# EcohydrologyTeam/ClearWater-riverine

Hardware: NVIDIA B200
Metric: cell_timesteps_per_sec (higher is better)
Workload: dtype f64

## Files before the change

clearwater_riverine_b200/csrc/cwr_api.cu:

```cuda
#include "../../include/cwr.h"

#include <cuda_runtime.h>

#include <algorithm>
#include <cmath>
#include <cstdio>
#include <cstdlib>
#include <cstring>
#include <map>
#include <string>
#include <vector>

#include "cwr_kernels.cuh"
#include "cwr_small.cuh"
#include "cwr_topology.h"

using namespace cwr;

static thread_local std::string g_create_error;

struct cwr_handle {
    int device = 0;
    cudaStream_t stream = nullptr;
    cwr_options opt{};
// ... 28 lines not shown
    int rank = 0, world = 1;
    bool attached = false;
    char* d_slab = nullptr; size_t slab_bytes = 0;
    uint8_t* d_send_mask = nullptr; int32_t* d_send_rows = nullptr;
    std::vector<void*> peer_maps;
    std::vector<int32_t> f1_ref, f2_ref;
    int last_iters = 0;
    bool small_path = false;
    bool tiny = false;
    int tiny_rpt = 1;
    int max_optin_smem = 0;
    bool pdl = false;
    int chip_ns = 0;
    bool in_run = false;
    SmallStats* d_stats = nullptr; SmallStats* h_stats = nullptr;
    int num_sms = 148, grid_rows = 0, grid_edges = 0, grid_b = 0, max_grid = 0, grid_spmm = 0, grid_at = 0, grid_xrp = 0;
    DeviceModel M{};
    int32_t *d_ell_col = nullptr, *d_ell_code = nullptr, *d_f1p = nullptr, *d_f2p = nullptr;
    int32_t *d_bcell = nullptr, *d_bptr = nullptr, *d_bedge = nullptr, *d_eperm = nullptr, *d_einv = nullptr;
    int32_t *d_new_of_old = nullptr, *d_old_of_new = nullptr, *d_f1 = nullptr, *d_f2 = nullptr;
    float *d_adv = nullptr, *d_velg = nullptr, *d_flowg = nullptr, *d_vol = nullptr;
    double* d_cdiff = nullptr;
    double* d_bc = nullptr;
    double* d_state = nullptr;
    double* d_dist = nullptr;
    void* d_stage = nullptr; size_t stage_bytes = 0;
    cudaStream_t up_stream = nullptr; cudaEvent_t compute_mark = nullptr;
    std::vector<cudaEvent_t> up_done; std::vector<uint8_t> up_pending;
    void* d_stage_up = nullptr; size_t stage_up_bytes = 0;
    cudaStream_t out_stream = nullptr; cudaEvent_t ev_extract[2] = {nullptr, nullptr}, ev_copied[2] = {nullptr, nullptr};
    double* d_out[2] = {nullptr, nullptr}; size_t out_bytes[2] = {0, 0}; int out_next = 0; bool out_pending[2] = {false, false};
    StepParams* d_sp = nullptr;
    StepParams* d_sp_ring = nullptr; size_t sp_ring_cap = 0; std::vector<StepParams> sp_host;
    const StepParams* sp_ready = nullptr;
    HostMirror* h_mirror = nullptr; HostMirror* d_mirror = nullptr;
    SolverCtl* h_ctl = nullptr;
    double* h_sc = nullptr; int* h_flags = nullptr;
    int n_state_slots = 0;
    std::vector<double> dt;
    std::vector<int> slot_time;
    std::vector<std::vector<double>> initial_row;
    std::vector<uint8_t> inputs_set;
    std::vector<std::map<int, std::vector<std::pair<int32_t, double>>>> real_overrides;
    int computed_upto = 0;
    int flux_step = -1;
    int lhs_step = -1;
    bool have_geometry = false;
    int64_t launches = 0, iterations = 0;
    bool kin_on = false;
    int kin_steps = 0, kin_temp_k = -1, kin_grid_max = 0;
    double kin_temp_c = 20.0;
    KinStep* d_kin_steps = nullptr; KinYield* d_kin_yields = nullptr; KinState* d_kin_state = nullptr; double* d_kin_partials = nullptr;
    int kin_srcs = 0, kin_src_o2 = 0;
    KinSrc* d_kin_srcs = nullptr;
    std::vector<double> kin_decay_h, kin_yields_h, kin_source_h, kin_exchange_h;
    std::vector<int> kin_step_of, kin_src_of;
    int kin_facs = 0;
    KinFac* d_kin_facs = nullptr; int* d_kin_fptr = nullptr;
    bool kin_depth = false;
    double kin_min_depth = 0.0;
    std::vector<double> kin_area_h;
// ... 151 lines not shown
    return v.empty() ? cudaSuccess : cudaMemcpyAsync(d, v.data(), v.size() * sizeof(T), cudaMemcpyHostToDevice, h->stream);
}

static int upload_kin_area(cwr_handle* h) {
    std::vector<double> a(h->n);
    for (int i = 0; i < h->n; ++i) a[i] = h->kin_area_h[h->topo.old_of_new[i]];
    CK(cudaMemcpyAsync(h->d_kin_area, a.data(), a.size() * sizeof(double), cudaMemcpyHostToDevice, h->stream));
    return CWR_OK;
}

static int upload_topology(cwr_handle* h) {
    const Topology& tp = h->topo;
    CK(put(h, h->d_ell_col, tp.ell_col)); CK(put(h, h->d_ell_code, tp.ell_code));
    CK(put(h, h->d_f1p, tp.f1p)); CK(put(h, h->d_f2p, tp.f2p));
    CK(put(h, h->d_bcell, tp.bcell)); CK(put(h, h->d_bptr, tp.bptr)); CK(put(h, h->d_bedge, tp.bedge));
    CK(put(h, h->d_eperm, tp.eperm));
    std::vector<int32_t> einv(tp.E);
    for (int ep = 0; ep < tp.E; ++ep) einv[tp.eperm[ep]] = ep;
    CK(put(h, h->d_einv, einv));
    CK(put(h, h->d_new_of_old, tp.new_of_old)); CK(put(h, h->d_old_of_new, tp.old_of_new));
    CK(put(h, h->d_color_ptr, tp.color_ptr));
    CK(put(h, h->d_send_mask, tp.send_mask)); CK(put(h, h->d_send_rows, tp.send_rows));
    if (h->strips) {
        CK(put(h, h->d_strip_cptr, tp.strip_cptr)); CK(put(h, h->d_strip_nptr, tp.strip_nptr));
        if (tp.strip_nbr.size() > h->strip_nbr_cap) {
            CK(cudaStreamSynchronize(h->stream));
            if (h->d_strip_nbr) CK(cudaFree(h->d_strip_nbr));
            h->d_strip_nbr = nullptr;
            h->strip_nbr_cap = tp.strip_nbr.size() + tp.strip_nbr.size() / 4 + 16;
            CK(cudaMalloc((void**)&h->d_strip_nbr, h->strip_nbr_cap * sizeof(int32_t)));
// ... 289 lines not shown
            CK(cudaFuncSetAttribute(k_solve_chip<12, false, true>, cudaFuncAttributeMaxDynamicSharedMemorySize, max_optin - kTinyStaticSmem));
            CK(cudaFuncSetAttribute(k_solve_chip<14, false, false>, cudaFuncAttributeMaxDynamicSharedMemorySize, max_optin - kTinyStaticSmem));
            CK(cudaFuncSetAttribute(k_solve_chip<14, false, true>, cudaFuncAttributeMaxDynamicSharedMemorySize, max_optin - kTinyStaticSmem));
            CK(cudaFuncSetAttribute(k_solve_chip<8, true, false>, cudaFuncAttributeMaxDynamicSharedMemorySize, max_optin - kTinyStaticSmem));
            CK(cudaFuncSetAttribute(k_solve_chip<8, true, true>, cudaFuncAttributeMaxDynamicSharedMemorySize, max_optin - kTinyStaticSmem));
            CK(cudaFuncSetAttribute(k_solve_chip<12, true, false>, cudaFuncAttributeMaxDynamicSharedMemorySize, max_optin - kTinyStaticSmem));
            CK(cudaFuncSetAttribute(k_solve_chip<12, true, true>, cudaFuncAttributeMaxDynamicSharedMemorySize, max_optin - kTinyStaticSmem));
            CK(cudaFuncSetAttribute(k_solve_chip<14, true, false>, cudaFuncAttributeMaxDynamicSharedMemorySize, max_optin - kTinyStaticSmem));
            CK(cudaFuncSetAttribute(k_solve_chip<14, true, true>, cudaFuncAttributeMaxDynamicSharedMemorySize, max_optin - kTinyStaticSmem));
            h->max_optin_smem = max_optin;
            choose_chip(h);
        }
    }
    h->grid_rows = grid_for(tp.part_ptr[h->rank + 1] - tp.part_ptr[h->rank], kThreads / kc, h->max_grid);
    h->grid_edges = grid_for(E / h->world + 1, kThreads / kc, h->max_grid);
    h->grid_b = grid_for((int64_t)(tp.bcell.size() / h->world + 1) * K, kThreads, h->max_grid);

    CK(dalloc(h, &h->d_ell_col, tp.ell_col.size())); CK(dalloc(h, &h->d_ell_code, tp.ell_code.size()));
    CK(dalloc(h, &h->d_f1p, tp.f1p.size())); CK(dalloc(h, &h->d_f2p, tp.f2p.size()));
    CK(dalloc(h, &h->d_bcell, tp.bcell.size())); CK(dalloc(h, &h->d_bptr, tp.bptr.size())); CK(dalloc(h, &h->d_bedge, tp.bedge.size()));
    CK(dalloc(h, &h->d_eperm, (size_t)E)); CK(dalloc(h, &h->d_einv, (size_t)E));
    CK(dalloc(h, &h->d_new_of_old, (size_t)n)); CK(dalloc(h, &h->d_old_of_new, (size_t)n));
    CK(dalloc(h, &h->d_color_ptr, tp.color_ptr.size()));
    CK(dalloc(h, &h->d_send_mask, (size_t)n)); CK(dalloc(h, &h->d_send_rows, (size_t)n));
    if (h->strips) {
        CK(dalloc(h, &h->d_strip_cptr, tp.strip_cptr.size())); CK(dalloc(h, &h->d_strip_nptr, tp.strip_nptr.size()));
        CK(dalloc(h, &h->d_strip_flag, (size_t)h->n_strips * kFlagStride));
        CK(cudaMemsetAsync(h->d_strip_flag, 0, (size_t)h->n_strips * kFlagStride * sizeof(unsigned long long), h->stream));
        CK(dalloc(h, &h->d_strip_peers, tp.strip_peers.size()));
        if ((size_t)h->world * h->n_strips * kFlagStride * sizeof(unsigned long long) > kDdCtlBytes - kDdFlagOffset)
            FAIL(CWR_EINVAL, "too many strips for the flag mirrors of a domain decomposition");
    }
    {
        int rc = upload_topology(h);
        if (rc) return rc;
// ... 11 lines not shown
    h->n_state_slots = h->opt.keep_history ? T : 2;
    const bool need_precond_vectors = h->m_steps > 1 || h->small_path;
    const size_t vec_bytes = (nK * sizeof(double) + 255) & ~(size_t)255;
    h->slab_bytes = kDdCtlBytes + (need_precond_vectors ? 3 : 0) * vec_bytes + (size_t)h->n_state_slots * nK * sizeof(double);
    if (cudaMalloc((void**)&h->d_slab, h->slab_bytes) != cudaSuccess) {
        cudaGetLastError();
        FAIL(CWR_ENOMEM, "not enough device memory for the concentration history; set keep_history = 0");
    }
    h->allocs.push_back(h->d_slab);
    CK(cudaMemsetAsync(h->d_slab, 0, h->slab_bytes, h->stream));
    h->d_state = (double*)(h->d_slab + kDdCtlBytes + (need_precond_vectors ? 3 : 0) * vec_bytes);

    DeviceModel& M = h->M;
    M.n = n; M.K = K; M.E = E; M.E_int = tp.E_int; M.E_g = tp.E_g; M.G = h->G; M.nb = (int)tp.bcell.size();
    M.W = tp.W; M.ell_col = h->d_ell_col; M.ell_code = h->d_ell_code; M.f1p = h->d_f1p; M.f2p = h->d_f2p;
    M.bcell = h->d_bcell; M.bptr = h->d_bptr; M.bedge = h->d_bedge;
    M.rank = h->rank; M.world = h->world;
    M.send_mask = h->d_send_mask;
    M.dd = (DdCtl*)h->d_slab; M.sym_base = h->d_slab;
    for (int q = 0; q < kMaxRanks; ++q) M.peer_base[q] = nullptr;
    M.peer_base[h->rank] = h->d_slab;
    set_owned_ranges(h);
    CK(dalloc(h, &M.val, (size_t)n * tp.W)); CK(dalloc(h, &M.diag, (size_t)n)); CK(dalloc(h, &M.gdiag, (size_t)n));
    CK(cudaMemsetAsync(M.gdiag, 0, (size_t)n * sizeof(double), h->stream));
    double* ic = nullptr;
    CK(dalloc(h, &ic, nK)); CK(cudaMemsetAsync(ic, 0, nK * sizeof(double), h->stream));
    M.ic = ic;
    CK(dalloc(h, &M.b, nK)); CK(dalloc(h, &M.r, nK));
    CK(cudaMemsetAsync(M.b, 0, nK * sizeof(double), h->stream)); CK(cudaMemsetAsync(M.r, 0, nK * sizeof(double), h->stream));
    {
        double** vs[] = {&M.rhat, &M.p, &M.v, &M.tt};
        for (double** v : vs) { CK(dalloc(h, v, nK)); CK(cudaMemsetAsync(*v, 0, nK * sizeof(double), h->stream)); }
    }
    if (need_precond_vectors) {
        double* us;
        CK(dalloc(h, &us, nK));
        CK(cudaMemsetAsync(us, 0, nK * sizeof(double), h->stream));
        M.ph = h->d_slab + kDdCtlBytes; M.sh = h->d_slab + kDdCtlBytes + vec_bytes; M.tmp = h->d_slab + kDdCtlBytes + 2 * vec_bytes;
        M.us = us;
// ... 263 lines not shown
}

static int state_available(cwr_handle* h, int t) {
    if (t < 0 || t >= h->T) FAIL(CWR_EINVAL, "time index out of range");
    if (t > h->computed_upto) FAIL(CWR_EINVAL, "state at this time index has not been computed yet");
    if (!h->opt.keep_history && t < h->computed_upto - 1) FAIL(CWR_EINVAL, "state no longer on the device (keep_history = 0)");
    return CWR_OK;
}

int cwr_set_state(cwr_handle* h, int k, int t, const double* c) {
    if (!h) return CWR_EINVAL;
    if (!c) FAIL(CWR_EINVAL, "NULL array");
    if (k < 0 || k >= h->K) FAIL(CWR_EINVAL, "constituent index out of range");
    int rc = state_available(h, t);
    if (rc) return rc;
    CK(cudaSetDevice(h->device));
    rc = ensure_stage(h, (size_t)h->n * 8);
    if (rc) return rc;
    CK(cudaMemcpyAsync(h->d_stage, c, (size_t)h->n * 8, cudaMemcpyHostToDevice, h->stream));
    k_scatter_column<<<grid_for(h->n, kThreads, h->max_grid), kThreads, 0, h->stream>>>(
        state_slot(h, t), (const double*)h->d_stage, h->d_old_of_new, h->n, h->K, k);
    h->launches += 1;
    CK(cudaGetLastError());
    CK(cudaStreamSynchronize(h->stream));
    return CWR_OK;
}

int cwr_set_state_all(cwr_handle* h, int t, const double* c, const uint8_t* mask) {
    if (!h) return CWR_EINVAL;
    if (!c) FAIL(CWR_EINVAL, "NULL array");
    int rc = state_available(h, t);
    if (rc) return rc;
    CK(cudaSetDevice(h->device));
    const size_t nK = (size_t)h->n * h->K;
    rc = ensure_stage(h, nK * 8 + 256);
    if (rc) return rc;
    uint8_t* dmask = nullptr;
    CK(cudaMemcpyAsync(h->d_stage, c, nK * 8, cudaMemcpyHostToDevice, h->stream));
    if (mask) {
        dmask = (uint8_t*)h->d_stage + nK * 8;
        CK(cudaMemcpyAsync(dmask, mask, h->K, cudaMemcpyHostToDevice, h->stream));
    }
    k_scatter_all<<<grid_for((int64_t)nK, kThreads, h->max_grid), kThreads, 0, h->stream>>>(
        state_slot(h, t), (const double*)h->d_stage, dmask, h->d_new_of_old, h->n, h->K);
    h->launches += 1;
    CK(cudaGetLastError());
    CK(cudaStreamSynchronize(h->stream));
// ... 111 lines not shown
        else if ((f & FL_BREAKDOWN) && !(f & FL_CONVERGED) && status == CWR_OK) status = CWR_EBREAKDOWN;
        else if (!(f & FL_CONVERGED) && status == CWR_OK) status = CWR_ENOTCONVERGED;
    }
    if (h->h_ctl->singular) status = CWR_ESINGULAR;
    if (h->h_ctl->barrier_timeout) { h->err = "a grid barrier timed out"; return CWR_ECUDA; }
    if (h->world > 1) {
        int dd_timeout = 0;
        CK(cudaMemcpyAsync(&dd_timeout, &h->M.dd->timeout, sizeof(int), cudaMemcpyDeviceToHost, h->stream));
        CK(cudaStreamSynchronize(h->stream));
        if (dd_timeout) { h->err = "a peer rank did not answer (halo barrier / dot-product exchange timed out)"; return CWR_ECUDA; }
    }
    if (info) { info->iterations = total_iter; info->restarts = restarts; info->status = status; info->max_relres = worst; }
    return status;
}

static int solve_dc(cwr_handle* h, cwr_step_info* info, bool* fell_back) {
    DeviceModel& M = h->M;
    *fell_back = false;
    mark(h, CWR_FAM_SPMM_INIT);
    KC_DISPATCH(h->KC, (k_spmm<KC, VEC, MODE_INIT_DC, double><<<h->grid_spmm, kThreads, 0, h->stream>>>(M, nullptr, nullptr)));
    h->launches += 1;
    mark(h, -1);
    int ahead = std::max(1, h->last_cycles);
    h->h_ctl->all_done = 0;
    int rc = CWR_OK;
    int launched = 0;
    while (!h->h_ctl->all_done) {
        const int burst = ahead > 0 ? ahead : h->opt.check_every;
        ahead = 0;
        for (int i = 0; i < burst; ++i) {
            const void* z = precondition(h, M.r, M.ph, M.tmp, true);
            mark(h, CWR_FAM_DC_UPDATE);
            PT_DISPATCH((k_spmm<KC, VEC, MODE_DC, PT><<<h->grid_spmm, kThreads, 0, h->stream>>>(M, (const PT*)z, nullptr)));
            h->launches += 1;
            ++launched;
// ... 77 lines not shown
    CK(cudaGetLastError());
    if (h->in_run) {
        if (info) { info->iterations = 0; info->restarts = 0; info->status = CWR_OK; info->max_relres = 0.0; }
        return CWR_OK;
    }
    int status = read_small_stats(h, info);
    if (status != CWR_ECUDA) h->iterations += (int64_t)(h->h_stats->sum_iterations / (unsigned long long)h->K);
    return status;
}

static int find_slot(cwr_handle* h, int t) {
    const int s = t % h->C;
    return h->slot_time[s] == t ? s : -1;
}

static int patch_real_cells(cwr_handle* h, int t, int before_solve) {
    DeviceModel& M = h->M;
    h->ov_idx.clear(); h->ov_val.clear();
    for (int k = 0; k < h->K; ++k) {
        auto it = h->real_overrides[k].find(t);
        if (it == h->real_overrides[k].end()) continue;
        for (auto& cv : it->second)
            if (cv.first >= M.row_lo && cv.first < M.row_hi) {
                h->ov_idx.push_back((long long)cv.first * h->K + k);
                h->ov_val.push_back(cv.second);
            }
    }
    const size_t cnt = h->ov_idx.size();
    if (cnt == 0) return CWR_OK;
    if (cnt > h->ov_cap) {
        CK(cudaStreamSynchronize(h->stream));
        if (h->d_ov_idx) CK(cudaFree(h->d_ov_idx));
        if (h->d_ov_val) CK(cudaFree(h->d_ov_val));
        h->d_ov_idx = nullptr; h->d_ov_val = nullptr;
        h->ov_cap = cnt + cnt / 2 + 64;
        CK(cudaMalloc((void**)&h->d_ov_idx, h->ov_cap * sizeof(long long)));
        CK(cudaMalloc((void**)&h->d_ov_val, h->ov_cap * sizeof(double)));
    }
    CK(cudaMemcpyAsync(h->d_ov_idx, h->ov_idx.data(), cnt * sizeof(long long), cudaMemcpyHostToDevice, h->stream));
    CK(cudaMemcpyAsync(h->d_ov_val, h->ov_val.data(), cnt * sizeof(double), cudaMemcpyHostToDevice, h->stream));
    CK(launch_chain(h, k_patch_rows, grid_for((int64_t)cnt, kThreads, 64), kThreads, 0, M, (const long long*)h->d_ov_idx, (const double*)h->d_ov_val, (int)cnt, before_solve));
    h->launches += 1;
    return CWR_OK;
}

static int build_rhs(cwr_handle* h, int t, int accumulate) {
    DeviceModel& M = h->M;
    mark(h, CWR_FAM_RHS);
    KC_DISPATCH(h->KC, (launch_chain(h, k_rhs<KC, VEC>, h->grid_rows, kThreads, 0, M)));
    h->launches += 1;
    int rc = patch_real_cells(h, t, 1);
    if (rc) return rc;
    if (h->kin_on) {
        const int R = react_tile_rows(h->K);
        const int grid = grid_for((M.row_hi - M.row_lo + R - 1) / R, 1, h->kin_grid_max);
        auto* fn = h->kin_depth ? k_react<true, true> : h->kin_facs ? k_react<true> : k_react<false>;
        const int* fptr = h->kin_depth && !h->kin_facs ? h->d_kin_fptr0 : h->d_kin_fptr;
        CK(launch_chain(h, fn, grid, kThreads, react_smem_bytes(h->K) + react_src_smem_bytes(h->kin_srcs, h->kin_temp_k), M,
                        (const KinStep*)h->d_kin_steps, h->kin_steps, (const KinYield*)h->d_kin_yields, h->kin_temp_k, h->kin_temp_c,
                        (const KinSrc*)h->d_kin_srcs, h->kin_srcs, h->kin_src_o2, (const KinFac*)h->d_kin_facs,
                        fptr, h->d_kin_partials, h->d_kin_state, accumulate, (const double*)h->d_kin_area,
                        (const int*)h->d_kin_dflag, h->kin_min_depth));
        h->launches += 1;
    }
    if (M.b_hi - M.b_lo > 0) {
        CK(launch_chain(h, k_boundary_rhs, h->grid_b, kThreads, 0, M));
        h->launches += 1;
    }
    return halo_push(h, h->cur_x);
}

static StepParams step_params(cwr_handle* h, int t, int s0, int s1) {
    const int n = h->n, E = h->E, K = h->K, Eg = std::max(1, h->topo.E_g), G = std::max(1, h->G);
    StepParams p;
    p.adv_t = h->d_adv + (size_t)s0 * E; p.cdiff_t = h->d_cdiff + (size_t)s0 * E;
    p.vol_t = h->d_vol + (size_t)s0 * n; p.vol_t1 = h->d_vol + (size_t)s1 * n;
    p.adv_t1 = h->d_adv + (size_t)s1 * E; p.cdiff_t1 = h->d_cdiff + (size_t)s1 * E;
    p.velg_t1 = h->d_velg + (size_t)s1 * Eg;
    p.flowg_t = h->d_flowg + (size_t)s0 * Eg;
    p.bc_t1 = h->d_bc + (size_t)(t + 1) * G * K;
    p.state_t = state_slot(h, t); p.state_t1 = state_slot(h, t + 1);
// ... 6 lines not shown
    if (t < 0 || t + 1 >= h->T) FAIL(CWR_EINVAL, "cwr_step: t must satisfy 0 <= t < n_time - 1 (dt[n_time-1] is NaN)");
    if (t > h->computed_upto) FAIL(CWR_EINVAL, "cwr_step: c[t] has not been computed yet");
    if (!h->opt.keep_history && t < h->computed_upto - 1) FAIL(CWR_EINVAL, "cwr_step: c[t] no longer on the device");
    for (int k = 0; k < h->K; ++k)
        if (!h->inputs_set[k]) FAIL(CWR_EINVAL, "cwr_set_inputs has not been called for every constituent");
    const int s0 = find_slot(h, t), s1 = find_slot(h, t + 1);
    if (s0 < 0 || s1 < 0) FAIL(CWR_EINVAL, "hydrodynamic slices t and t+1 are not resident; call cwr_set_hydro");
    CK(cudaSetDevice(h->device));
    { int rcj = join_prefetch(h, s0); if (rcj) return rcj; rcj = join_prefetch(h, s1); if (rcj) return rcj; }
    const int64_t launches0 = h->launches;
    const StepParams p = step_params(h, t, s0, s1);
    DeviceModel& M = h->M;
    if (h->sp_ready) M.sp = const_cast<StepParams*>(h->sp_ready);
    else CK(launch_chain(h, k_set_step, 1, 1, 0, p, h->d_sp, M.ctl, h->world > 1 ? M.dd : (DdCtl*)nullptr));
    h->cur_x = p.state_t1;
    mark(h, CWR_FAM_ASSEMBLE);
    if (h->world > 1 && !h->attached) FAIL(CWR_EINVAL, "domain-decomposed handle: call cwr_dd_attach before stepping");
    const int nb_own = M.b_hi - M.b_lo;
    if (nb_own > 0) CK(launch_chain(h, k_boundary_diag, grid_for(nb_own, kThreads, h->max_grid), kThreads, 0, M));
    CK(launch_chain(h, k_assemble, grid_for(M.row_hi - M.row_lo, kThreads, h->max_grid), kThreads, 0, M));
    h->launches += 2 + (nb_own > 0);
    h->lhs_step = t;
    { int rc = build_rhs(h, t, 1); if (rc) return rc; }
    cwr_step_info local{};
    int status;
    if (h->small_path) status = solve_small(h, &local);
    else if (h->dc) {
        bool fell_back = false;
        status = solve_dc(h, &local, &fell_back);
        if (fell_back) {
            ++h->fallbacks;
            const int cycles = h->h_ctl->iter, sweeps = h->h_ctl->sweeps_done;
            CK(cudaMemsetAsync(&M.ctl->all_done, 0, 2 * sizeof(int), h->stream));
            h->last_iters = 0;
            { int rc = build_rhs(h, t, 0); if (rc) return rc; }
            status = solve(h, &local);
            local.restarts += 1 + cycles;
            local.sweeps = sweeps;
        }
    } else status = solve(h, &local);
    if (status == CWR_ECUDA) return status;
    { int rc = patch_real_cells(h, t + 1, 0); if (rc) return rc; }
    { int rc = halo_push(h, p.state_t1); if (rc) return rc; }
    if (M.want_flux) {
        mark(h, CWR_FAM_MASS_FLUX);
        KC_DISPATCH(h->KC, (launch_chain(h, k_mass_flux<KC, VEC>, h->grid_edges, kThreads, 0, M)));
        h->launches += 1;
        h->flux_step = t;
    }
    flush_profile(h);
    CK(cudaGetLastError());
    h->computed_upto = std::max(h->computed_upto, t + 1);
    if (!h->opt.keep_history) h->computed_upto = t + 1;
    local.n_launches = (int)(h->launches - launches0);
    if (info) *info = local;
    if (status != CWR_OK) {
        char buf[160];
// ... 564 lines not shown
            const double v = pr.second < 0 ? diag[i] : val[pr.second] * diag[i];
            if (pr.first == last) data[pos - 1] += v;
            else { indices[pos] = pr.first; data[pos] = v; ++pos; last = pr.first; }
        }
    }
    indptr[n] = (int32_t)pos;
    return CWR_OK;
}

int cwr_get_rhs(cwr_handle* h, int k, double* b) {
    if (!h) return CWR_EINVAL;
    if (!b) FAIL(CWR_EINVAL, "NULL array");
    if (k < 0 || k >= h->K) FAIL(CWR_EINVAL, "constituent index out of range");
    if (h->lhs_step < 0) FAIL(CWR_EINVAL, "no step taken yet");
    CK(cudaSetDevice(h->device));
    const int n = h->n, K = h->K;
    std::vector<double> bs((size_t)n * K), diag(n);
    CK(cudaMemcpyAsync(bs.data(), h->M.b, bs.size() * 8, cudaMemcpyDeviceToHost, h->stream));
    CK(cudaMemcpyAsync(diag.data(), h->M.diag, (size_t)n * 8, cudaMemcpyDeviceToHost, h->stream));
    CK(cudaStreamSynchronize(h->stream));
    for (int r0 = 0; r0 < n; ++r0) {
        const int i = h->topo.new_of_old[r0];
        b[r0] = bs[(size_t)i * K + k] * diag[i];
    }
    return CWR_OK;
}

int cwr_get_permutation(cwr_handle* h, int32_t* new_of_old) {
    if (!h) return CWR_EINVAL;
    if (!new_of_old) FAIL(CWR_EINVAL, "NULL array");
// ... 161 lines not shown
```

clearwater_riverine_b200/csrc/cwr_kernels.cuh:

```cuda
#pragma once
#include <cuda_runtime.h>
#include <stdint.h>

#include "cwr_topology.h"

namespace cwr {

constexpr int kThreads = 256;
constexpr int kMaxK = 128;
constexpr int kMaxDots = 4;
#ifndef CWR_SPMM_MIN_BLOCKS
#define CWR_SPMM_MIN_BLOCKS 4
#endif
#ifndef CWR_AT_MIN_BLOCKS
#define CWR_AT_MIN_BLOCKS 3
#endif

struct StepParams {
    const float* adv_t;
    const double* cdiff_t;
    const float* vol_t;
    const float* vol_t1;
    const float* adv_t1;
    const double* cdiff_t1;
// ... 49 lines not shown
struct DeviceModel {
    int n, K, E, E_int, E_g, G, nb, W;
    int row_lo, row_hi, ie_lo, ie_hi, ge_lo, ge_hi, b_lo, b_hi;
    int rank, world;
    unsigned nbr_mask;
    const uint8_t* send_mask;
    const int32_t* send_rows; int n_send;
    int halo_per_sweep;
    char* peer_base[kMaxRanks];
    char* sym_base;
    DdCtl* dd;
    const int32_t* ell_col;
    const int32_t* ell_code;
    const int32_t* f1p; const int32_t* f2p;
    const int32_t* bcell; const int32_t* bptr; const int32_t* bedge;
    const int32_t* color_ptr; int n_colors;
    const int32_t* strip_cptr; const int32_t* strip_nptr; const int32_t* strip_nbr;
    const uint8_t* strip_peers;
    unsigned long long* strip_flag;
    int n_strips, strip0;
    int us_from_producer;
    int sweep_f32;
    int dc_smin, dc_smax;
    double dc_floor;
    double* val;
    float* valf;
    double* diag;
    double* gdiag;
    const double* ic;
    double *b, *r, *rhat, *p, *v, *tt, *xc;
    void *ph, *sh, *tmp, *us;
    double* partials;
    double* sc;
    int* colflags;
    int* coliters;
    SolverCtl* ctl;
    const StepParams* sp;
    double* flux;
    double* bsum;
    double* vsum;
    double tol2;
    double diffusion_coefficient;
    int max_iter;
// ... 114 lines not shown
        float ad = __fmul_rn(area, Df);
        adv[ep] = a;
        cdiff[ep] = (double)ad / dist[e];
        if (ep >= E_int) { velg[ep - E_int] = u; flowg[ep - E_int] = q; }
    }
}

__global__ void k_dist(double* __restrict__ dist, const double* __restrict__ fx, const double* __restrict__ fy,
                       const int32_t* __restrict__ f1, const int32_t* __restrict__ f2, int E) {
    for (int e = blockIdx.x * blockDim.x + threadIdx.x; e < E; e += gridDim.x * blockDim.x) {
        double dx = fx[f1[e]] - fx[f2[e]], dy = fy[f1[e]] - fy[f2[e]];
        dist[e] = sqrt(__dadd_rn(__dmul_rn(dx, dx), __dmul_rn(dy, dy)));
    }
}

__global__ void k_boundary_diag(DeviceModel M) {
    pdl_enter();
    const StepParams& sp = *M.sp;
    for (int b = M.b_lo + blockIdx.x * blockDim.x + threadIdx.x; b < M.b_hi; b += gridDim.x * blockDim.x) {
        double s = 0.0;
        for (int j = M.bptr[b]; j < M.bptr[b + 1]; ++j) {
            int e = M.bedge[j];
            s += sp.cdiff_t[e] + fmax((double)sp.adv_t[e], 0.0);
        }
        M.gdiag[M.bcell[b]] = s;
    }
}

__global__ void __launch_bounds__(kThreads) k_assemble(DeviceModel M) {
    pdl_enter();
    const StepParams& sp = *M.sp;
    const double dt = sp.dt;
    const int W = M.W;
    for (int i = M.row_lo + blockIdx.x * blockDim.x + threadIdx.x; i < M.row_hi; i += gridDim.x * blockDim.x) {
        const float vol = sp.vol_t1[i];
        double diag = (vol == 0.f ? 1.0 : 0.0) + (double)vol / dt + M.gdiag[i];
        const int32_t* code = M.ell_code + (size_t)i * W;
        double* val = M.val + (size_t)i * W;
        if (W == 4) {
            const int4 c4 = *reinterpret_cast<const int4*>(code);
            const int cs[4] = {c4.x, c4.y, c4.z, c4.w};
            double a[4], d[4], off[4];
#pragma unroll
            for (int u = 0; u < 4; ++u) {
                a[u] = cs[u] >= 0 ? (double)sp.adv_t[cs[u] >> 1] : 0.0;
                d[u] = cs[u] >= 0 ? sp.cdiff_t[cs[u] >> 1] : 0.0;
            }
#pragma unroll
            for (int u = 0; u < 4; ++u) {
                off[u] = 0.0;
                if (cs[u] >= 0) {
// ... 43 lines not shown
template <int VEC> struct Vd { double a[VEC]; };

template <int VEC>
__device__ __forceinline__ Vd<VEC> ldv(const double* p) {
    Vd<VEC> r;
    if (VEC == 2) { const double2 t = *reinterpret_cast<const double2*>(p); r.a[0] = t.x; r.a[VEC - 1] = t.y; }
    else r.a[0] = *p;
    return r;
}
template <int VEC>
__device__ __forceinline__ void stv(double* p, const Vd<VEC>& v) {
    if (VEC == 2) *reinterpret_cast<double2*>(p) = make_double2(v.a[0], v.a[VEC - 1]);
    else *p = v.a[0];
}

template <int KC, int VEC>
__global__ void __launch_bounds__(kThreads) k_rhs(DeviceModel M) {
    pdl_enter();
    const StepParams& sp = *M.sp;
    const int K = M.K, lane = threadIdx.x % KC, group = threadIdx.x / KC, GPB = kThreads / KC;
    const double dt = sp.dt;
    for (int c = lane * VEC; c < K; c += KC * VEC)
        for (int i = M.row_lo + blockIdx.x * GPB + group; i < M.row_hi; i += gridDim.x * GPB) {
            const size_t idx = (size_t)i * K + c;
            Vd<VEC> conc = ldv<VEC>(sp.state_t + idx);
            if (sp.apply_ic) {
                const Vd<VEC> ic = ldv<VEC>(M.ic + idx);
#pragma unroll
                for (int q = 0; q < VEC; ++q) if (ic.a[q] != 0.0) conc.a[q] = ic.a[q];
            }
            const double vol = (double)sp.vol_t[i], dg = M.diag[i];
            Vd<VEC> bb;
#pragma unroll
            for (int q = 0; q < VEC; ++q) bb.a[q] = (vol * conc.a[q] / dt) / dg;
            stv<VEC>(M.b + idx, bb);
            stv<VEC>(sp.state_t1 + idx, conc);
        }
}

__global__ void k_patch_rows(DeviceModel M, const long long* __restrict__ idx, const double* __restrict__ val, int count, int before_solve) {
    pdl_enter();
    const StepParams& sp = *M.sp;
    for (int q = blockIdx.x * blockDim.x + threadIdx.x; q < count; q += gridDim.x * blockDim.x) {
        const long long i = idx[q];
        const int row = (int)(i / M.K);
        sp.state_t1[i] = val[q];
        if (before_solve) M.b[i] = ((double)sp.vol_t[row] * val[q] / sp.dt) / M.diag[row];
    }
}

__global__ void __launch_bounds__(kThreads) k_boundary_rhs(DeviceModel M) {
    pdl_enter();
    const StepParams& sp = *M.sp;
    const int K = M.K;
    const double dt = sp.dt;
    const bool has_diffusion = M.diffusion_coefficient != 0.0;
    const size_t total = (size_t)(M.b_hi - M.b_lo) * K;
    for (size_t q = blockIdx.x * (size_t)blockDim.x + threadIdx.x; q < total; q += (size_t)gridDim.x * blockDim.x) {
        const int b = M.b_lo + (int)(q / K), c = (int)(q % K);
        const int i = M.bcell[b];
        double m_in = 0.0, ca_in = 0.0, cd_in = 0.0, m_out = 0.0, cd_out = 0.0;
        for (int j = M.bptr[b]; j < M.bptr[b + 1]; ++j) {
            const int e = M.bedge[j];
            const float u = sp.velg_t1[e - M.E_int];
            const double bc = sp.bc_t1[(size_t)(M.f2p[e] - M.n) * K + c];
            const double cd = has_diffusion ? fabs(sp.cdiff_t1[e]) : 0.0;
            if (u < 0.f) { m_in = bc; ca_in = fabs((double)sp.adv_t1[e]); cd_in = cd; }
            if (u > 0.f) { m_out = bc; cd_out = cd; }
        }
        const size_t idx = (size_t)i * K + c;
        const double conc = sp.state_t1[idx];
        const double load = (double)sp.vol_t[i] * conc / dt;
        const double rhs = load + (ca_in + cd_in) * m_in + cd_out * m_out;
        M.b[idx] = rhs / M.diag[i];
    }
}

template <int ND, int KC, int VEC>
__device__ __forceinline__ void block_dots(double (&acc)[ND * VEC], double* smem, double* partials, int K, int chunk) {
    constexpr int NA = ND * VEC;
#pragma unroll
    for (int off = KC; off < 32; off <<= 1)
#pragma unroll
        for (int d = 0; d < NA; ++d) acc[d] += __shfl_xor_sync(0xffffffffu, acc[d], off);
    const int wl = threadIdx.x & 31, warp = threadIdx.x >> 5;
    constexpr int NW = kThreads / 32;
    if (wl < KC)
#pragma unroll
        for (int d = 0; d < NA; ++d) smem[(warp * NA + d) * KC + wl] = acc[d];
    __syncthreads();
// ... 1142 lines not shown

template <int KC, int VEC, int MODE, typename ZT>
__global__ void __launch_bounds__(kThreads, MODE == 2 ? CWR_AT_MIN_BLOCKS : CWR_SPMM_MIN_BLOCKS) k_spmm(DeviceModel M, const ZT* __restrict__ zin,
                                                                        double* __restrict__ out) {
    constexpr bool IS_INIT = MODE == MODE_INIT || MODE == MODE_INIT_DC;
    constexpr int ND = IS_INIT ? 2 : MODE == MODE_AV ? 1 : MODE == MODE_AT ? 4 : 1;
    constexpr bool HAS_DOTS = IS_INIT || MODE == MODE_AV || MODE == MODE_AT || MODE == MODE_DC;
    __shared__ double smem[HAS_DOTS ? (kThreads / 32) * kMaxDots * 2 * 32 : 1];
    __shared__ double tot[HAS_DOTS ? kMaxDots * kMaxK : 1];
    if (MODE == MODE_AV || MODE == MODE_AT || MODE == MODE_DC) { if (M.ctl->all_done) return; }
    if (MODE == MODE_AT) { if (M.ctl->finish_half) return; }
    const int K = M.K, n = M.row_hi, W = M.W;
    const int lane = threadIdx.x % KC, group = threadIdx.x / KC, GPB = kThreads / KC;
    const int32_t* __restrict__ ecol = M.ell_col;
    const double* __restrict__ eval = M.val;
    if (IS_INIT) zin = reinterpret_cast<const ZT*>(M.sp->state_t1);
    double* __restrict__ xs = M.sp->state_t1;
    const int nchunk = (K + KC * VEC - 1) / (KC * VEC);
    for (int chunk = 0; chunk < nchunk; ++chunk) {
        const int c = (chunk * KC + lane) * VEC;
        const bool active = c < K;
        double acc[ND * VEC];
#pragma unroll
        for (int d = 0; d < ND * VEC; ++d) acc[d] = 0.0;
        if (active) {
            const int stride = gridDim.x * GPB;
            int i = M.row_lo + blockIdx.x * GPB + group;
            int4 c4n = make_int4(0, 0, 0, 0);
            double2 v01n = make_double2(0.0, 0.0), v23n = v01n;
            if (i < n) {
                c4n = *reinterpret_cast<const int4*>(ecol + (size_t)i * W);
                v01n = *reinterpret_cast<const double2*>(eval + (size_t)i * W);
                v23n = *reinterpret_cast<const double2*>(eval + (size_t)i * W + 2);
            }
            for (; i < n; i += stride) {
                const size_t idx = (size_t)i * K + c;
                const int4 c4 = make_int4(c4n.x & kColMask, c4n.y & kColMask, c4n.z & kColMask, c4n.w & kColMask);
                const double2 v01 = v01n, v23 = v23n;
                const Vd<VEC> x0 = ldz<ZT, VEC>(zin + (size_t)c4.x * K + c);
                const Vd<VEC> x1 = ldz<ZT, VEC>(zin + (size_t)c4.y * K + c);
                const Vd<VEC> x2 = ldz<ZT, VEC>(zin + (size_t)c4.z * K + c);
                const Vd<VEC> x3 = ldz<ZT, VEC>(zin + (size_t)c4.w * K + c);
                const Vd<VEC> own = ldz<ZT, VEC>(zin + idx);
                Vd<VEC> aux1 = own, aux2 = own;
                if (IS_INIT) aux1 = ldv<VEC>(M.b + idx);
                if (MODE == MODE_AV || MODE == MODE_AT) aux1 = ldv<VEC>(M.rhat + idx);
                if (MODE == MODE_DC) { aux1 = ldv<VEC>(M.r + idx); aux2 = ldv<VEC>(xs + idx); }
                if (MODE == MODE_AT) aux2 = ldv<VEC>(M.r + idx);
                const int inext = i + stride;
                if (inext < n) {
                    c4n = *reinterpret_cast<const int4*>(ecol + (size_t)inext * W);
                    v01n = *reinterpret_cast<const double2*>(eval + (size_t)inext * W);
                    v23n = *reinterpret_cast<const double2*>(eval + (size_t)inext * W + 2);
                }
                Vd<VEC> s;
#pragma unroll
                for (int q = 0; q < VEC; ++q)
                    s.a[q] = fma(v23.y, x3.a[q], fma(v23.x, x2.a[q], fma(v01.y, x1.a[q], v01.x * x0.a[q])));
                for (int w = 4; w < W; w += 4) {
                    int4 d4 = *reinterpret_cast<const int4*>(ecol + (size_t)i * W + w);
                    d4.x &= kColMask; d4.y &= kColMask; d4.z &= kColMask; d4.w &= kColMask;
                    const double2 w01 = *reinterpret_cast<const double2*>(eval + (size_t)i * W + w);
                    const double2 w23 = *reinterpret_cast<const double2*>(eval + (size_t)i * W + w + 2);
                    const Vd<VEC> y0 = ldz<ZT, VEC>(zin + (size_t)d4.x * K + c);
                    const Vd<VEC> y1 = ldz<ZT, VEC>(zin + (size_t)d4.y * K + c);
                    const Vd<VEC> y2 = ldz<ZT, VEC>(zin + (size_t)d4.z * K + c);
                    const Vd<VEC> y3 = ldz<ZT, VEC>(zin + (size_t)d4.w * K + c);
#pragma unroll
                    for (int q = 0; q < VEC; ++q)
                        s.a[q] = fma(w23.y, y3.a[q], fma(w23.x, y2.a[q], fma(w01.y, y1.a[q], fma(w01.x, y0.a[q], s.a[q]))));
                }
                Vd<VEC> y;
#pragma unroll
                for (int q = 0; q < VEC; ++q) y.a[q] = own.a[q] + s.a[q];
                if (IS_INIT) {
                    const Vd<VEC> bi = aux1;
                    Vd<VEC> r;
#pragma unroll
                    for (int q = 0; q < VEC; ++q) {
                        r.a[q] = bi.a[q] - y.a[q];
                        acc[0 * VEC + q] = fma(r.a[q], r.a[q], acc[0 * VEC + q]);
                        acc[1 * VEC + q] = fma(bi.a[q], bi.a[q], acc[1 * VEC + q]);
                    }
                    stv<VEC>(M.r + idx, r);
                    if (MODE == MODE_INIT) { stv<VEC>(M.rhat + idx, r); stv<VEC>(M.p + idx, r); }
                    if (MODE == MODE_INIT_DC && M.us_from_producer) {
                        if (M.sweep_f32) {
                            Pk<float, VEC> rs;
#pragma unroll
                            for (int q = 0; q < VEC; ++q) rs.a[q] = (float)r.a[q];
                            stk<float, VEC>(reinterpret_cast<float*>(M.us) + idx, rs);
                        } else stv<VEC>(reinterpret_cast<double*>(M.us) + idx, r);
                    }
                } else if (MODE == MODE_DC) {
                    Vd<VEC> r = aux1, xv = aux2;
#pragma unroll
                    for (int q = 0; q < VEC; ++q) {
                        r.a[q] -= y.a[q];
                        xv.a[q] += own.a[q];
                        acc[q] = fma(r.a[q], r.a[q], acc[q]);
                    }
                    stv<VEC>(M.r + idx, r); stv<VEC>(xs + idx, xv);
                    if (M.us_from_producer) {
                        Pk<ZT, VEC> rs;
#pragma unroll
                        for (int q = 0; q < VEC; ++q) rs.a[q] = (ZT)r.a[q];
                        stk<ZT, VEC>(reinterpret_cast<ZT*>(M.us) + idx, rs);
// ... 343 lines not shown
```

Measured before the change: 8.756 billion.

## Fuse RHS formation and boundary terms into assembly and DC initial SpMM

Removes the separate boundary-diagonal and boundary-RHS kernels. Ghost diagonal contributions are now computed inside k_assemble through a new cell-to-boundary-row map, and the RHS is formed on the fly in the MODE_INIT_DC SpMM from c[t] instead of being written to b and read back. On the direct path the state copy into t+1 is done by the SpMM itself, so several launches and one full pass over b and the state are dropped. In exchange cwr_get_rhs must recompute b lazily and fails if c[t] has been evicted, and edge-value prefetching is disabled in the init-DC mode.

```diff
diff --git a/clearwater_riverine_b200/csrc/cwr_api.cu b/clearwater_riverine_b200/csrc/cwr_api.cu
--- a/clearwater_riverine_b200/csrc/cwr_api.cu
+++ b/clearwater_riverine_b200/csrc/cwr_api.cu
@@ -66,10 +66,10 @@
     int chip_ns = 0;
     bool in_run = false;
     SmallStats* d_stats = nullptr; SmallStats* h_stats = nullptr;
-    int num_sms = 148, grid_rows = 0, grid_edges = 0, grid_b = 0, max_grid = 0, grid_spmm = 0, grid_at = 0, grid_xrp = 0;
+    int num_sms = 148, grid_rows = 0, grid_edges = 0, max_grid = 0, grid_spmm = 0, grid_at = 0, grid_xrp = 0;
     DeviceModel M{};
     int32_t *d_ell_col = nullptr, *d_ell_code = nullptr, *d_f1p = nullptr, *d_f2p = nullptr;
-    int32_t *d_bcell = nullptr, *d_bptr = nullptr, *d_bedge = nullptr, *d_eperm = nullptr, *d_einv = nullptr;
+    int32_t *d_bcell = nullptr, *d_bptr = nullptr, *d_bedge = nullptr, *d_brow = nullptr, *d_eperm = nullptr, *d_einv = nullptr;
     int32_t *d_new_of_old = nullptr, *d_old_of_new = nullptr, *d_f1 = nullptr, *d_f2 = nullptr;
     float *d_adv = nullptr, *d_velg = nullptr, *d_flowg = nullptr, *d_vol = nullptr;
     double* d_cdiff = nullptr;
@@ -97,6 +97,7 @@
     int computed_upto = 0;
     int flux_step = -1;
     int lhs_step = -1;
+    bool rhs_direct = false, rhs_lost = false;
     bool have_geometry = false;
     int64_t launches = 0, iterations = 0;
     bool kin_on = false;
@@ -278,6 +279,9 @@
     CK(put(h, h->d_ell_col, tp.ell_col)); CK(put(h, h->d_ell_code, tp.ell_code));
     CK(put(h, h->d_f1p, tp.f1p)); CK(put(h, h->d_f2p, tp.f2p));
     CK(put(h, h->d_bcell, tp.bcell)); CK(put(h, h->d_bptr, tp.bptr)); CK(put(h, h->d_bedge, tp.bedge));
+    std::vector<int32_t> brow(tp.n, -1);
+    for (size_t b = 0; b < tp.bcell.size(); ++b) brow[tp.bcell[b]] = (int32_t)b;
+    CK(put(h, h->d_brow, brow));
     CK(put(h, h->d_eperm, tp.eperm));
     std::vector<int32_t> einv(tp.E);
     for (int ep = 0; ep < tp.E; ++ep) einv[tp.eperm[ep]] = ep;
@@ -597,11 +601,11 @@
     }
     h->grid_rows = grid_for(tp.part_ptr[h->rank + 1] - tp.part_ptr[h->rank], kThreads / kc, h->max_grid);
     h->grid_edges = grid_for(E / h->world + 1, kThreads / kc, h->max_grid);
-    h->grid_b = grid_for((int64_t)(tp.bcell.size() / h->world + 1) * K, kThreads, h->max_grid);
 
     CK(dalloc(h, &h->d_ell_col, tp.ell_col.size())); CK(dalloc(h, &h->d_ell_code, tp.ell_code.size()));
     CK(dalloc(h, &h->d_f1p, tp.f1p.size())); CK(dalloc(h, &h->d_f2p, tp.f2p.size()));
     CK(dalloc(h, &h->d_bcell, tp.bcell.size())); CK(dalloc(h, &h->d_bptr, tp.bptr.size())); CK(dalloc(h, &h->d_bedge, tp.bedge.size()));
+    CK(dalloc(h, &h->d_brow, (size_t)tp.n));
     CK(dalloc(h, &h->d_eperm, (size_t)E)); CK(dalloc(h, &h->d_einv, (size_t)E));
     CK(dalloc(h, &h->d_new_of_old, (size_t)n)); CK(dalloc(h, &h->d_old_of_new, (size_t)n));
     CK(dalloc(h, &h->d_color_ptr, tp.color_ptr.size()));
@@ -643,15 +647,14 @@
     DeviceModel& M = h->M;
     M.n = n; M.K = K; M.E = E; M.E_int = tp.E_int; M.E_g = tp.E_g; M.G = h->G; M.nb = (int)tp.bcell.size();
     M.W = tp.W; M.ell_col = h->d_ell_col; M.ell_code = h->d_ell_code; M.f1p = h->d_f1p; M.f2p = h->d_f2p;
-    M.bcell = h->d_bcell; M.bptr = h->d_bptr; M.bedge = h->d_bedge;
+    M.bcell = h->d_bcell; M.bptr = h->d_bptr; M.bedge = h->d_bedge; M.brow = h->d_brow;
     M.rank = h->rank; M.world = h->world;
     M.send_mask = h->d_send_mask;
     M.dd = (DdCtl*)h->d_slab; M.sym_base = h->d_slab;
     for (int q = 0; q < kMaxRanks; ++q) M.peer_base[q] = nullptr;
     M.peer_base[h->rank] = h->d_slab;
     set_owned_ranges(h);
-    CK(dalloc(h, &M.val, (size_t)n * tp.W)); CK(dalloc(h, &M.diag, (size_t)n)); CK(dalloc(h, &M.gdiag, (size_t)n));
-    CK(cudaMemsetAsync(M.gdiag, 0, (size_t)n * sizeof(double), h->stream));
+    CK(dalloc(h, &M.val, (size_t)n * tp.W)); CK(dalloc(h, &M.diag, (size_t)n));
     double* ic = nullptr;
     CK(dalloc(h, &ic, nK)); CK(cudaMemsetAsync(ic, 0, nK * sizeof(double), h->stream));
     M.ic = ic;
@@ -945,6 +948,7 @@
     if (k < 0 || k >= h->K) FAIL(CWR_EINVAL, "constituent index out of range");
     int rc = state_available(h, t);
     if (rc) return rc;
+    if (t == h->lhs_step) h->rhs_lost = true;
     CK(cudaSetDevice(h->device));
     rc = ensure_stage(h, (size_t)h->n * 8);
     if (rc) return rc;
@@ -962,6 +966,7 @@
     if (!c) FAIL(CWR_EINVAL, "NULL array");
     int rc = state_available(h, t);
     if (rc) return rc;
+    if (t == h->lhs_step) h->rhs_lost = true;
     CK(cudaSetDevice(h->device));
     const size_t nK = (size_t)h->n * h->K;
     rc = ensure_stage(h, nK * 8 + 256);
@@ -1103,11 +1108,12 @@
     return status;
 }
 
-static int solve_dc(cwr_handle* h, cwr_step_info* info, bool* fell_back) {
+static int solve_dc(cwr_handle* h, cwr_step_info* info, bool* fell_back, const double* c_tilde) {
     DeviceModel& M = h->M;
     *fell_back = false;
     mark(h, CWR_FAM_SPMM_INIT);
-    KC_DISPATCH(h->KC, (k_spmm<KC, VEC, MODE_INIT_DC, double><<<h->grid_spmm, kThreads, 0, h->stream>>>(M, nullptr, nullptr)));
+    double* b_out = h->rhs_direct ? nullptr : M.b;
+    KC_DISPATCH(h->KC, (k_spmm<KC, VEC, MODE_INIT_DC, double><<<h->grid_spmm, kThreads, 0, h->stream>>>(M, c_tilde, b_out)));
     h->launches += 1;
     mark(h, -1);
     int ahead = std::max(1, h->last_cycles);
@@ -1215,7 +1221,7 @@
     return h->slot_time[s] == t ? s : -1;
 }
 
-static int patch_real_cells(cwr_handle* h, int t, int before_solve) {
+static int patch_real_cells(cwr_handle* h, int t) {
     DeviceModel& M = h->M;
     h->ov_idx.clear(); h->ov_val.clear();
     for (int k = 0; k < h->K; ++k) {
@@ -1240,17 +1246,27 @@
     }
     CK(cudaMemcpyAsync(h->d_ov_idx, h->ov_idx.data(), cnt * sizeof(long long), cudaMemcpyHostToDevice, h->stream));
     CK(cudaMemcpyAsync(h->d_ov_val, h->ov_val.data(), cnt * sizeof(double), cudaMemcpyHostToDevice, h->stream));
-    CK(launch_chain(h, k_patch_rows, grid_for((int64_t)cnt, kThreads, 64), kThreads, 0, M, (const long long*)h->d_ov_idx, (const double*)h->d_ov_val, (int)cnt, before_solve));
+    CK(launch_chain(h, k_patch_rows, grid_for((int64_t)cnt, kThreads, 64), kThreads, 0, M, (const long long*)h->d_ov_idx, (const double*)h->d_ov_val, (int)cnt));
     h->launches += 1;
     return CWR_OK;
 }
 
-static int build_rhs(cwr_handle* h, int t, int accumulate) {
+static bool has_real_overrides(const cwr_handle* h, int t) {
+    for (int k = 0; k < h->K; ++k)
+        if (h->real_overrides[k].count(t)) return true;
+    return false;
+}
+
+static int front_end(cwr_handle* h, int t, bool direct, bool form_b, int accumulate) {
     DeviceModel& M = h->M;
+    mark(h, CWR_FAM_ASSEMBLE);
+    CK(launch_chain(h, k_assemble, grid_for(M.row_hi - M.row_lo, kThreads, h->max_grid), kThreads, 0, M, direct ? 0 : 1));
+    h->launches += 1;
+    h->lhs_step = t;
+    h->rhs_direct = direct; h->rhs_lost = false;
+    if (direct) return CWR_OK;
     mark(h, CWR_FAM_RHS);
-    KC_DISPATCH(h->KC, (launch_chain(h, k_rhs<KC, VEC>, h->grid_rows, kThreads, 0, M)));
-    h->launches += 1;
-    int rc = patch_real_cells(h, t, 1);
+    int rc = patch_real_cells(h, t);
     if (rc) return rc;
     if (h->kin_on) {
         const int R = react_tile_rows(h->K);
@@ -1264,8 +1280,8 @@
                         (const int*)h->d_kin_dflag, h->kin_min_depth));
         h->launches += 1;
     }
-    if (M.b_hi - M.b_lo > 0) {
-        CK(launch_chain(h, k_boundary_rhs, h->grid_b, kThreads, 0, M));
+    if (form_b) {
+        KC_DISPATCH(h->KC, (launch_chain(h, k_rhs<KC, VEC>, h->grid_rows, kThreads, 0, M, (const double*)h->cur_x)));
         h->launches += 1;
     }
     return halo_push(h, h->cur_x);
@@ -1302,33 +1318,28 @@
     if (h->sp_ready) M.sp = const_cast<StepParams*>(h->sp_ready);
     else CK(launch_chain(h, k_set_step, 1, 1, 0, p, h->d_sp, M.ctl, h->world > 1 ? M.dd : (DdCtl*)nullptr));
     h->cur_x = p.state_t1;
-    mark(h, CWR_FAM_ASSEMBLE);
     if (h->world > 1 && !h->attached) FAIL(CWR_EINVAL, "domain-decomposed handle: call cwr_dd_attach before stepping");
-    const int nb_own = M.b_hi - M.b_lo;
-    if (nb_own > 0) CK(launch_chain(h, k_boundary_diag, grid_for(nb_own, kThreads, h->max_grid), kThreads, 0, M));
-    CK(launch_chain(h, k_assemble, grid_for(M.row_hi - M.row_lo, kThreads, h->max_grid), kThreads, 0, M));
-    h->launches += 2 + (nb_own > 0);
-    h->lhs_step = t;
-    { int rc = build_rhs(h, t, 1); if (rc) return rc; }
+    const bool direct = h->dc && h->world == 1 && t >= 1 && !h->kin_on && !has_real_overrides(h, t);
+    { int rc = front_end(h, t, direct, !h->dc, 1); if (rc) return rc; }
     cwr_step_info local{};
     int status;
     if (h->small_path) status = solve_small(h, &local);
     else if (h->dc) {
         bool fell_back = false;
-        status = solve_dc(h, &local, &fell_back);
+        status = solve_dc(h, &local, &fell_back, direct ? p.state_t : p.state_t1);
         if (fell_back) {
             ++h->fallbacks;
             const int cycles = h->h_ctl->iter, sweeps = h->h_ctl->sweeps_done;
             CK(cudaMemsetAsync(&M.ctl->all_done, 0, 2 * sizeof(int), h->stream));
             h->last_iters = 0;
-            { int rc = build_rhs(h, t, 0); if (rc) return rc; }
+            { int rc = front_end(h, t, false, true, 0); if (rc) return rc; }
             status = solve(h, &local);
             local.restarts += 1 + cycles;
             local.sweeps = sweeps;
         }
     } else status = solve(h, &local);
     if (status == CWR_ECUDA) return status;
-    { int rc = patch_real_cells(h, t + 1, 0); if (rc) return rc; }
+    { int rc = patch_real_cells(h, t + 1); if (rc) return rc; }
     { int rc = halo_push(h, p.state_t1); if (rc) return rc; }
     if (M.want_flux) {
         mark(h, CWR_FAM_MASS_FLUX);
@@ -1923,6 +1934,14 @@
     if (k < 0 || k >= h->K) FAIL(CWR_EINVAL, "constituent index out of range");
     if (h->lhs_step < 0) FAIL(CWR_EINVAL, "no step taken yet");
     CK(cudaSetDevice(h->device));
+    if (h->rhs_direct) {
+        const int t = h->lhs_step;
+        if (h->rhs_lost || state_available(h, t) != CWR_OK || find_slot(h, t) < 0 || find_slot(h, t + 1) < 0)
+            FAIL(CWR_EINVAL, "cwr_get_rhs: c[t] or the hydrodynamic slices t, t+1 of the last step are no longer on the device");
+        KC_DISPATCH(h->KC, (launch_chain(h, k_rhs<KC, VEC>, h->grid_rows, kThreads, 0, h->M, (const double*)state_slot(h, t))));
+        h->launches += 1;
+        CK(cudaGetLastError());
+    }
     const int n = h->n, K = h->K;
     std::vector<double> bs((size_t)n * K), diag(n);
     CK(cudaMemcpyAsync(bs.data(), h->M.b, bs.size() * 8, cudaMemcpyDeviceToHost, h->stream));
diff --git a/clearwater_riverine_b200/csrc/cwr_kernels.cuh b/clearwater_riverine_b200/csrc/cwr_kernels.cuh
--- a/clearwater_riverine_b200/csrc/cwr_kernels.cuh
+++ b/clearwater_riverine_b200/csrc/cwr_kernels.cuh
@@ -87,6 +87,7 @@
     const int32_t* ell_code;
     const int32_t* f1p; const int32_t* f2p;
     const int32_t* bcell; const int32_t* bptr; const int32_t* bedge;
+    const int32_t* brow;
     const int32_t* color_ptr; int n_colors;
     const int32_t* strip_cptr; const int32_t* strip_nptr; const int32_t* strip_nbr;
     const uint8_t* strip_peers;
@@ -99,7 +100,6 @@
     double* val;
     float* valf;
     double* diag;
-    double* gdiag;
     const double* ic;
     double *b, *r, *rhat, *p, *v, *tt, *xc;
     void *ph, *sh, *tmp, *us;
@@ -244,27 +244,38 @@
     }
 }
 
-__global__ void k_boundary_diag(DeviceModel M) {
-    pdl_enter();
-    const StepParams& sp = *M.sp;
-    for (int b = M.b_lo + blockIdx.x * blockDim.x + threadIdx.x; b < M.b_hi; b += gridDim.x * blockDim.x) {
-        double s = 0.0;
-        for (int j = M.bptr[b]; j < M.bptr[b + 1]; ++j) {
-            int e = M.bedge[j];
-            s += sp.cdiff_t[e] + fmax((double)sp.adv_t[e], 0.0);
-        }
-        M.gdiag[M.bcell[b]] = s;
-    }
-}
-
-__global__ void __launch_bounds__(kThreads) k_assemble(DeviceModel M) {
+__global__ void __launch_bounds__(kThreads) k_assemble(DeviceModel M, int with_x0) {
     pdl_enter();
     const StepParams& sp = *M.sp;
     const double dt = sp.dt;
     const int W = M.W;
+    if (with_x0) {
+        const size_t lo = (size_t)M.row_lo * M.K, hi = (size_t)M.row_hi * M.K, stride = (size_t)gridDim.x * blockDim.x;
+        const double* __restrict__ src = sp.state_t;
+        double* __restrict__ dst = sp.state_t1;
+        for (size_t q = lo + blockIdx.x * (size_t)blockDim.x + threadIdx.x; q < hi; q += 2 * stride) {
+            const size_t q1 = q + stride;
+            double v0 = src[q], v1 = q1 < hi ? src[q1] : 0.0;
+            if (sp.apply_ic) {
+                const double i0 = M.ic[q], i1 = q1 < hi ? M.ic[q1] : 0.0;
+                if (i0 != 0.0) v0 = i0;
+                if (i1 != 0.0) v1 = i1;
+            }
+            dst[q] = v0;
+            if (q1 < hi) dst[q1] = v1;
+        }
+    }
     for (int i = M.row_lo + blockIdx.x * blockDim.x + threadIdx.x; i < M.row_hi; i += gridDim.x * blockDim.x) {
         const float vol = sp.vol_t1[i];
-        double diag = (vol == 0.f ? 1.0 : 0.0) + (double)vol / dt + M.gdiag[i];
+        const double own = (vol == 0.f ? 1.0 : 0.0) + (double)vol / dt;
+        const int bi = M.brow[i];
+        double ghost = 0.0;
+        if (bi >= 0)
+            for (int j = M.bptr[bi]; j < M.bptr[bi + 1]; ++j) {
+                const int e = M.bedge[j];
+                ghost += sp.cdiff_t[e] + fmax((double)sp.adv_t[e], 0.0);
+            }
+        double diag = own + ghost;
         const int32_t* code = M.ell_code + (size_t)i * W;
         double* val = M.val + (size_t)i * W;
         if (W == 4) {
@@ -338,8 +349,44 @@
     else *p = v.a[0];
 }
 
+template <int VEC>
+__device__ __forceinline__ Vd<VEC> rhs_row(const DeviceModel& M, const StepParams& sp, int bi, int c, const Vd<VEC>& conc,
+                                           float vol, double dg, double dt) {
+    Vd<VEC> b;
+#pragma unroll
+    for (int q = 0; q < VEC; ++q) b.a[q] = __dmul_rn((double)vol, conc.a[q]) / dt;
+    if (bi >= 0) {
+        int e_in = -1, e_out = -1;
+        for (int j = M.bptr[bi]; j < M.bptr[bi + 1]; ++j) {
+            const int e = M.bedge[j];
+            const float u = sp.velg_t1[e - M.E_int];
+            if (u < 0.f) e_in = e;
+            if (u > 0.f) e_out = e;
+        }
+        const bool has_diffusion = M.diffusion_coefficient != 0.0;
+        double cin = 0.0, cd_out = 0.0;
+        const double* bc_in = nullptr; const double* bc_out = nullptr;
+        if (e_in >= 0) {
+            cin = __dadd_rn(fabs((double)sp.adv_t1[e_in]), has_diffusion ? fabs(sp.cdiff_t1[e_in]) : 0.0);
+            bc_in = sp.bc_t1 + (size_t)(M.f2p[e_in] - M.n) * M.K + c;
+        }
+        if (e_out >= 0) {
+            cd_out = has_diffusion ? fabs(sp.cdiff_t1[e_out]) : 0.0;
+            bc_out = sp.bc_t1 + (size_t)(M.f2p[e_out] - M.n) * M.K + c;
+        }
+#pragma unroll
+        for (int q = 0; q < VEC; ++q) {
+            const double m_in = bc_in ? bc_in[q] : 0.0, m_out = bc_out ? bc_out[q] : 0.0;
+            b.a[q] = __dadd_rn(__dadd_rn(b.a[q], __dmul_rn(cin, m_in)), __dmul_rn(cd_out, m_out));
+        }
+    }
+#pragma unroll
+    for (int q = 0; q < VEC; ++q) b.a[q] = b.a[q] / dg;
+    return b;
+}
+
 template <int KC, int VEC>
-__global__ void __launch_bounds__(kThreads) k_rhs(DeviceModel M) {
+__global__ void __launch_bounds__(kThreads) k_rhs(DeviceModel M, const double* __restrict__ src) {
     pdl_enter();
     const StepParams& sp = *M.sp;
     const int K = M.K, lane = threadIdx.x % KC, group = threadIdx.x / KC, GPB = kThreads / KC;
@@ -347,57 +394,15 @@
     for (int c = lane * VEC; c < K; c += KC * VEC)
         for (int i = M.row_lo + blockIdx.x * GPB + group; i < M.row_hi; i += gridDim.x * GPB) {
             const size_t idx = (size_t)i * K + c;
-            Vd<VEC> conc = ldv<VEC>(sp.state_t + idx);
-            if (sp.apply_ic) {
-                const Vd<VEC> ic = ldv<VEC>(M.ic + idx);
-#pragma unroll
-                for (int q = 0; q < VEC; ++q) if (ic.a[q] != 0.0) conc.a[q] = ic.a[q];
-            }
-            const double vol = (double)sp.vol_t[i], dg = M.diag[i];
-            Vd<VEC> bb;
-#pragma unroll
-            for (int q = 0; q < VEC; ++q) bb.a[q] = (vol * conc.a[q] / dt) / dg;
-            stv<VEC>(M.b + idx, bb);
-            stv<VEC>(sp.state_t1 + idx, conc);
-        }
-}
-
-__global__ void k_patch_rows(DeviceModel M, const long long* __restrict__ idx, const double* __restrict__ val, int count, int before_solve) {
+            const Vd<VEC> conc = ldv<VEC>(src + idx);
+            stv<VEC>(M.b + idx, rhs_row<VEC>(M, sp, M.brow[i], c, conc, sp.vol_t[i], M.diag[i], dt));
+        }
+}
+
+__global__ void k_patch_rows(DeviceModel M, const long long* __restrict__ idx, const double* __restrict__ val, int count) {
     pdl_enter();
     const StepParams& sp = *M.sp;
-    for (int q = blockIdx.x * blockDim.x + threadIdx.x; q < count; q += gridDim.x * blockDim.x) {
-        const long long i = idx[q];
-        const int row = (int)(i / M.K);
-        sp.state_t1[i] = val[q];
-        if (before_solve) M.b[i] = ((double)sp.vol_t[row] * val[q] / sp.dt) / M.diag[row];
-    }
-}
-
-__global__ void __launch_bounds__(kThreads) k_boundary_rhs(DeviceModel M) {
-    pdl_enter();
-    const StepParams& sp = *M.sp;
-    const int K = M.K;
-    const double dt = sp.dt;
-    const bool has_diffusion = M.diffusion_coefficient != 0.0;
-    const size_t total = (size_t)(M.b_hi - M.b_lo) * K;
-    for (size_t q = blockIdx.x * (size_t)blockDim.x + threadIdx.x; q < total; q += (size_t)gridDim.x * blockDim.x) {
-        const int b = M.b_lo + (int)(q / K), c = (int)(q % K);
-        const int i = M.bcell[b];
-        double m_in = 0.0, ca_in = 0.0, cd_in = 0.0, m_out = 0.0, cd_out = 0.0;
-        for (int j = M.bptr[b]; j < M.bptr[b + 1]; ++j) {
-            const int e = M.bedge[j];
-            const float u = sp.velg_t1[e - M.E_int];
-            const double bc = sp.bc_t1[(size_t)(M.f2p[e] - M.n) * K + c];
-            const double cd = has_diffusion ? fabs(sp.cdiff_t1[e]) : 0.0;
-            if (u < 0.f) { m_in = bc; ca_in = fabs((double)sp.adv_t1[e]); cd_in = cd; }
-            if (u > 0.f) { m_out = bc; cd_out = cd; }
-        }
-        const size_t idx = (size_t)i * K + c;
-        const double conc = sp.state_t1[idx];
-        const double load = (double)sp.vol_t[i] * conc / dt;
-        const double rhs = load + (ca_in + cd_in) * m_in + cd_out * m_out;
-        M.b[idx] = rhs / M.diag[i];
-    }
+    for (int q = blockIdx.x * blockDim.x + threadIdx.x; q < count; q += gridDim.x * blockDim.x) sp.state_t1[idx[q]] = val[q];
 }
 
 template <int ND, int KC, int VEC>
@@ -1570,8 +1575,10 @@
     const int lane = threadIdx.x % KC, group = threadIdx.x / KC, GPB = kThreads / KC;
     const int32_t* __restrict__ ecol = M.ell_col;
     const double* __restrict__ eval = M.val;
-    if (IS_INIT) zin = reinterpret_cast<const ZT*>(M.sp->state_t1);
+    if (MODE == MODE_INIT) zin = reinterpret_cast<const ZT*>(M.sp->state_t1);
     double* __restrict__ xs = M.sp->state_t1;
+    const double dt = M.sp->dt;
+    const float* __restrict__ vol_t = M.sp->vol_t;
     const int nchunk = (K + KC * VEC - 1) / (KC * VEC);
     for (int chunk = 0; chunk < nchunk; ++chunk) {
         const int c = (chunk * KC + lane) * VEC;
@@ -1580,34 +1587,44 @@
 #pragma unroll
         for (int d = 0; d < ND * VEC; ++d) acc[d] = 0.0;
         if (active) {
+            constexpr bool PREFETCH_VALUES = MODE != MODE_INIT_DC;
             const int stride = gridDim.x * GPB;
             int i = M.row_lo + blockIdx.x * GPB + group;
             int4 c4n = make_int4(0, 0, 0, 0);
             double2 v01n = make_double2(0.0, 0.0), v23n = v01n;
             if (i < n) {
                 c4n = *reinterpret_cast<const int4*>(ecol + (size_t)i * W);
-                v01n = *reinterpret_cast<const double2*>(eval + (size_t)i * W);
-                v23n = *reinterpret_cast<const double2*>(eval + (size_t)i * W + 2);
+                if (PREFETCH_VALUES) {
+                    v01n = *reinterpret_cast<const double2*>(eval + (size_t)i * W);
+                    v23n = *reinterpret_cast<const double2*>(eval + (size_t)i * W + 2);
+                }
             }
             for (; i < n; i += stride) {
                 const size_t idx = (size_t)i * K + c;
                 const int4 c4 = make_int4(c4n.x & kColMask, c4n.y & kColMask, c4n.z & kColMask, c4n.w & kColMask);
-                const double2 v01 = v01n, v23 = v23n;
+                const double2 v01 = PREFETCH_VALUES ? v01n : *reinterpret_cast<const double2*>(eval + (size_t)i * W);
+                const double2 v23 = PREFETCH_VALUES ? v23n : *reinterpret_cast<const double2*>(eval + (size_t)i * W + 2);
                 const Vd<VEC> x0 = ldz<ZT, VEC>(zin + (size_t)c4.x * K + c);
                 const Vd<VEC> x1 = ldz<ZT, VEC>(zin + (size_t)c4.y * K + c);
                 const Vd<VEC> x2 = ldz<ZT, VEC>(zin + (size_t)c4.z * K + c);
                 const Vd<VEC> x3 = ldz<ZT, VEC>(zin + (size_t)c4.w * K + c);
                 const Vd<VEC> own = ldz<ZT, VEC>(zin + idx);
                 Vd<VEC> aux1 = own, aux2 = own;
-                if (IS_INIT) aux1 = ldv<VEC>(M.b + idx);
+                if (MODE == MODE_INIT) aux1 = ldv<VEC>(M.b + idx);
+                int brw = -1;
+                float vol = 0.f;
+                double dg = 1.0;
+                if (MODE == MODE_INIT_DC) { brw = M.brow[i]; vol = vol_t[i]; dg = M.diag[i]; }
                 if (MODE == MODE_AV || MODE == MODE_AT) aux1 = ldv<VEC>(M.rhat + idx);
                 if (MODE == MODE_DC) { aux1 = ldv<VEC>(M.r + idx); aux2 = ldv<VEC>(xs + idx); }
                 if (MODE == MODE_AT) aux2 = ldv<VEC>(M.r + idx);
                 const int inext = i + stride;
                 if (inext < n) {
                     c4n = *reinterpret_cast<const int4*>(ecol + (size_t)inext * W);
-                    v01n = *reinterpret_cast<const double2*>(eval + (size_t)inext * W);
-                    v23n = *reinterpret_cast<const double2*>(eval + (size_t)inext * W + 2);
+                    if (PREFETCH_VALUES) {
+                        v01n = *reinterpret_cast<const double2*>(eval + (size_t)inext * W);
+                        v23n = *reinterpret_cast<const double2*>(eval + (size_t)inext * W + 2);
+                    }
                 }
                 Vd<VEC> s;
 #pragma unroll
@@ -1630,7 +1647,7 @@
 #pragma unroll
                 for (int q = 0; q < VEC; ++q) y.a[q] = own.a[q] + s.a[q];
                 if (IS_INIT) {
-                    const Vd<VEC> bi = aux1;
+                    const Vd<VEC> bi = MODE == MODE_INIT_DC ? rhs_row<VEC>(M, *M.sp, brw, c, own, vol, dg, dt) : aux1;
                     Vd<VEC> r;
 #pragma unroll
                     for (int q = 0; q < VEC; ++q) {
@@ -1647,6 +1664,10 @@
                             for (int q = 0; q < VEC; ++q) rs.a[q] = (float)r.a[q];
                             stk<float, VEC>(reinterpret_cast<float*>(M.us) + idx, rs);
                         } else stv<VEC>(reinterpret_cast<double*>(M.us) + idx, r);
+                    }
+                    if (MODE == MODE_INIT_DC) {
+                        if (out) stv<VEC>(out + idx, bi);
+                        else stv<VEC>(xs + idx, own);
                     }
                 } else if (MODE == MODE_DC) {
                     Vd<VEC> r = aux1, xv = aux2;
```

Result: faster. 9.092 billion (median of 6 runs) (+3.8%).
